# The-Learning-And-Vision-Atelier-LAVA/BUFFER

Hardware: AMD Instinct MI355X
Metric: registration pairs/sec (higher is better)
Workload: dtype f32

## Files before the change

buffer_amd/_lib.py:

```python
import ctypes as C
import os

_HERE = os.path.dirname(os.path.abspath(__file__))
LIB_PATH = os.environ.get("BUF_LIB_PATH") or os.path.join(_HERE, "libbuffer_hip.so")

BUF_OK = 0


class BufferHipError(RuntimeError):
    pass


class buf_grid_t(C.Structure):
    _fields_ = [
        ("ws", C.c_void_p), ("ws_bytes", C.c_size_t),
        ("ns", C.c_int), ("nb", C.c_int),
        ("cells_per_elem", C.c_int64),
        ("radius", C.c_float),
        ("supports", C.c_void_p),
        ("desc", C.c_void_p), ("s_off", C.c_void_p), ("table", C.c_void_p),
        ("sorted", C.c_void_p), ("order", C.c_void_p), ("scan_tmp", C.c_void_p),
    ]


# ... 37 lines not shown
    "buf_vn_gather_block_pre": (_i, [_vp, _vp, _vp, _vp, _i, _i, _i, _i, _i, _f, _vp, _vp, _vp, _vp, _f, _vp, _vp, _sz, _vp]),
    "buf_vn_pointwise": (_i, [_vp, _vp, _i, _i, _i, _vp, _i, _i, _i, _vp, _vp, _vp, _vp, _f, _vp, _vp, _vp]),
    "buf_gather_max": (_i, [_vp, _vp, _i, _i, _i, _i, _vp, _vp]),
    "buf_vn_std": (_i, [_vp, _vp, _i, _i, _vp, _vp]),
    "buf_score_head_ws_bytes": (_sz, [_i, _i]),
    "buf_score_head": (_i, [_vp, _i, _vp, _i, _vp, _vp, _vp, _vp, _f, _vp, _vp, _vp, _vp, _f, _vp, _vp, _vp, _vp, _vp, _i, _vp, _vp, _i, _f,
                            _vp, _vp, _sz, _vp]),
    "buf_patch_voxelize_ws_bytes": (_sz, [_i]),
    "buf_patch_voxelize": (_i, [_vp, _vp, _i, _i, _f, _vp, _i, _i, _vp, _f, _i, _vp, _vp, _vp, _vp, _vp, _vp, _vp,
                                _vp, _vp, _sz, _vp]),
    "buf_cylindrical_net_wg": (_i, [_vp, _i, _vp, _vp, _vp, _vp, _vp, _vp, _vp]),
    "buf_cylindrical_net_wg_supports": (_i, [_vp, _vp]),
    "buf_cylindrical_net_split_safe": (_i, [_vp, _i, _vp, _vp, _vp, _vp, _vp, _vp, _vp, _vp, _vp, _vp, _vp, _vp]),
    "buf_cost_volume_net_split_safe": (_i, [_vp, _vp, _i, _vp, _vp, _i, _vp, _vp, _vp, _vp, _vp, _vp, _vp, _vp]),
    "buf_cylindrical_net_split": (_i, [_vp, _i, _vp, _vp, _vp, _vp, _vp, _vp, _vp, _vp]),
    "buf_cylindrical_net_split_head": (_i, [_vp, _i, _vp, _vp, _vp, _vp, _vp, _vp, _vp, _vp, _vp, _vp]),
    "buf_split_gemm_count": (C.c_longlong, [_i, _i, _i, _i]),
    "buf_split_tile_gemm": (_i, [_vp, _i, _i, _i, _i, _vp]),
    "buf_cost_volume_net_split": (_i, [_vp, _vp, _i, _vp, _vp, _vp, _vp, _vp]),
    "buf_cost_volume_net_split_gather": (_i, [_vp, _i, _vp, _vp, _i, _vp, _vp, _vp, _vp, _vp]),
    "buf_split_filter_count": (C.c_longlong, [_i, _i]),
    "buf_split_tile_filters": (_i, [_vp, _i, _i, _vp]),
    "buf_winograd_tile_weights": (_i, [_vp, _i, _i, _vp]),
    "buf_winograd_group": (_i, [_i, _i]),
    "buf_cost_winograd_group": (_i, [_i]),
    "buf_winograd_tile_filters": (_i, [_vp, _i, _i, _i, _i, _vp]),
    "buf_voxel_downsample_ws_bytes": (_sz, [_i, _i64]),
    "buf_voxel_downsample": (_i, [_vp, _vp, _i, _i, C.c_double, _vp, _vp, _vp, _i64, _vp, _sz, _vp]),
    "buf_voxel_downsample_batch_ws_bytes": (_sz, [_i, _i, _i64]),
    "buf_voxel_downsample_batch": (_i, [_vp, _i, _i, _vp, _i, C.c_double, _vp, _vp, _i64, _vp, _sz, _vp]),
    "buf_knn_normals": (_i, [_vp, _i, _vp, _i, _vp, _i, _i, _vp, _i, _vp, _vp, _vp]),
    "buf_icp_ws_bytes": (_sz, [_i, _i, _i, _i]),
    "buf_icp_batched": (_i, [_vp, _vp, _vp, _vp, _vp, _i, _i, _f, _vp, _i, C.c_double, C.c_double, _vp, _vp, _vp, _vp, _vp,
                             _vp, _sz, _vp]),
    "buf_pair_stats_ws_bytes": (_sz, [_i, _i, _i, _i, _i64]),
    "buf_pair_stats": (_i, [_vp, _vp, _i, _vp, _vp, _i, _vp, _f, _i64, _vp, _vp, _vp, _vp, _sz, _vp]),
    "buf_match_metrics": (_i, [_vp, _vp, _vp, _i, _i, _vp, _vp, _f, _f, _f, _vp, _vp, _vp]),
    "buf_row_linear": (_i, [_vp, _i, _i, _i, _vp, _vp, _i, _vp, _vp]),
    "buf_segment_instance_norm_ws_bytes": (_sz, [_i, _i]),
    "buf_segment_instance_norm": (_i, [_vp, _i, _i, _vp, _i, _f, _vp, _vp, _sz, _vp]),
    "buf_descriptor_head": (_i, [_vp, _i, _vp, _vp, _vp, _vp]),
    "buf_cost_volume_net": (_i, [_vp, _vp, _i, _vp, _vp, _vp, _vp]),
    "buf_cost_volume_net_gather": (_i, [_vp, _i, _vp, _vp, _i, _vp, _vp, _vp, _vp]),
    "buf_hypotheses_score": (_i, [_vp, _vp, _vp, _vp, _vp, _i, _i, _f, _vp, _vp, _vp, _vp, _vp, _vp]),
    "buf_ransac_ws_bytes": (_sz, [_i]),
    "buf_ransac_kabsch": (_i, [_vp, _vp, _vp, _i, _i, C.c_uint64, _f, _f, _vp, _vp, _vp, _sz, _vp]),
# ... 34 lines not shown
```

buffer_amd/csrc/buffer_hip.hip:

```cpp
#include <stdlib.h>
#include "core.hip"
#include "radius.hip"
#include "icp.hip"
#include "pairstats.hip"
#include "metrics.hip"
#include "subsample.hip"
#include "pointops.hip"
#include "vn.hip"
#include "voxelize.hip"
#include "registration.hip"
#include "convnet.hip"
#include "convnet_h3.hip"
#include "costnet_h3.hip"
#include "preprocess.hip"
#include "convnet_wg.hip"
#include "costnet.hip"
#include "split_safe.hip"
```

buffer_amd/csrc/convnet_wg.hip:

```cpp
#include "common.h"
#include <type_traits>

#define WG_CS 160
#define WG_ROW 22
#define WG_ZERO 154
#define WG_MAXC 128
#define WG_LAYERS 8
#define WG_THREADS 256
#define WG_BUF (WG_MAXC * WG_CS)
#define WG_KSTEP (16 * WG_CS)
#define WG_BLOCKS 16

typedef float wgf4 __attribute__((ext_vector_type(4)));
typedef float wgf2 __attribute__((ext_vector_type(2)));
typedef const __attribute__((address_space(3))) wgf2* wg_lds_f2;

struct CylWgParams {
    const float* wt[WG_LAYERS];
    const float* bias[WG_LAYERS];
    int cin[WG_LAYERS], cout[WG_LAYERS], relu[WG_LAYERS];
    const int* only_if;
#ifdef WG_STAMP
    long long* stamps;
#endif
// ... 464 lines not shown
    wg_first_weights<2, 0, 2>(rs, wp, lofs, wstride, W1);
    float park[2][3][16];
    wg_round<2, 0, 2>(RA, rs, wp, wp, lofs, k4 >> 2, wstride, pstride, bv, W1, Y);
    wg_park<0>(Y, park);
    wg_park<1>(Y, park);
    wgf4 Yb[2];
    wg_round_direct<2>(RA[2][0], rs, wp, lofs, k4 >> 2, wstride, pstride, bv, W1, Yb);
    Y[0][2][0][0] = Yb[0]; Y[1][2][0][0] = Yb[1];
    wg_park<2>(Y, park);
    __syncthreads();
    int lane_s = threadIdx.x & (WAVE - 1);
    asm volatile("" : "+v"(lane_s));
#pragma unroll
    for (int n = 0; n < 2; n++) {
#pragma unroll
        for (int t = 0; t < 3; t++)
#pragma unroll
            for (int q = 0; q < (t == 2 ? 4 : 16); q++)
                asm volatile("v_accvgpr_read_b32 %0, %1" : "=v"(Y[n][t][q >> 3][(q >> 2) & 1][q & 3]) : "a"(park[n][t][q]));
        wg_store(Y[n], 2 * pair + n, relu, act, lane_s & 15, lane_s >> 4);
    }
}

__device__ __forceinline__ void cyl_net_wg_body(const float* __restrict__ x, const CylWgParams& P, float* __restrict__ y, float* __restrict__ lds)
{
    float* act = lds;
    const int patch = blockIdx.x;
    const int w = __builtin_amdgcn_readfirstlane(threadIdx.x / WAVE);
    WG_STAMP_AT(17)
#ifdef WG_STAMP
    if (threadIdx.x == 0) { P.stamps[(size_t)gridDim.x * 80 + blockIdx.x * 4 + 0] = __builtin_amdgcn_s_memtime(); P.stamps[(size_t)gridDim.x * 80 + blockIdx.x * 4 + 1] = __builtin_amdgcn_s_memrealtime(); }
#endif
    {
        const wgf4* src = reinterpret_cast<const wgf4*>(x + (size_t)patch * P.cin[0] * 140);
        const int nq = P.cin[0] * 35;
        wgf4 v[8];
#pragma unroll
        for (int k = 0; k < 8; k++) {
            const int i = threadIdx.x + k * WG_THREADS;
            if (i < nq) v[k] = __builtin_nontemporal_load(src + i);
        }
        auto put = [&](int i, wgf4 u) __attribute__((always_inline)) {
            const int c = i / 35, q = i - c * 35;
            const int row = q / 5, col = (q - row * 5) * 4;
            float* p = act + c * WG_CS + row * WG_ROW + col + 1;
            p[0] = u[0]; p[1] = u[1]; p[2] = u[2]; p[3] = u[3];
            if (col == 0) p[20] = u[0];
            if (col == 16) p[-17] = u[3];
        };
#pragma unroll
        for (int k = 0; k < 8; k++) {
            const int i = threadIdx.x + k * WG_THREADS;
            if (i < nq) put(i, v[k]);
        }
        for (int i = threadIdx.x + 8 * WG_THREADS; i < nq; i += WG_THREADS) put(i, __builtin_nontemporal_load(src + i));
    }
    for (int i = threadIdx.x; i < WG_MAXC * 4; i += WG_THREADS) act[(i >> 2) * WG_CS + WG_ZERO + (i & 3)] = 0.f;
    __syncthreads();
    WG_STAMP_AT(0)
    WgAddrPark pk;
    {
        int lane0 = threadIdx.x & (WAVE - 1);
        asm volatile("" : "+v"(lane0));
        wg_park_addresses(act, lane0 & 15, lane0 >> 4, pk);
    }
#pragma unroll 1
    for (int l = 0; l < WG_LAYERS; l++) {
        const int cin = P.cin[l], cout = P.cout[l];
        if (cout == 128) wg_layer_pair(act, P.wt[l], P.bias[l], cin, cout, P.relu[l], w, pk);
        else if (cout == 64) wg_layer_msplit(act, P.wt[l], P.bias[l], cin, cout, P.relu[l], w, pk);
        else if (l < WG_LAYERS - 1) wg_layer_mksplit<false>(act, nullptr, P.wt[l], P.bias[l], cin, cout, P.relu[l], w, pk);
        else wg_layer_mksplit<true>(act, y + (size_t)patch * cout * 140, P.wt[l], P.bias[l], cin, cout, P.relu[l], w, pk);
        WG_STAMP_AT(2 * l + 1)
        __syncthreads();
        WG_STAMP_AT(2 * l + 2)
    }
#ifdef WG_STAMP
    if (threadIdx.x == 0) { P.stamps[(size_t)gridDim.x * 80 + blockIdx.x * 4 + 2] = __builtin_amdgcn_s_memtime(); P.stamps[(size_t)gridDim.x * 80 + blockIdx.x * 4 + 3] = __builtin_amdgcn_s_memrealtime(); }
#endif
}

// ... 47 lines not shown
{
    for (int l = 0; l < WG_LAYERS; l++) {
        const int ci = cin[l], co = cout[l];
        BUF_REQUIRE(ci > 0 && ci % 16 == 0 && ci <= WG_MAXC && (co == 32 || co == 64 || co == 128), BUF_EINVAL,
                    "buf_cylindrical_net_wg: layer %d has unsupported widths %d -> %d", l, ci, co);
        BUF_REQUIRE(co != 128 || ci % 32 == 0, BUF_EINVAL,
                    "buf_cylindrical_net_wg: layer %d has unsupported widths %d -> %d (128 output channels need Cin %% 32 == 0)", l, ci, co);
        BUF_REQUIRE(co != 32 || (ci % 32 == 0 && ci <= 64), BUF_EINVAL,
                    "buf_cylindrical_net_wg: layer %d has unsupported widths %d -> %d (32 output channels need Cin = 32 or 64)", l, ci, co);
        BUF_REQUIRE(l == 0 || ci == cout[l - 1], BUF_EINVAL, "buf_cylindrical_net_wg: layer %d width mismatch", l);
        BUF_REQUIRE(l == 0 || cout[l - 1] != 32 || co == 32, BUF_EINVAL,
                    "buf_cylindrical_net_wg: layer %d has unsupported widths %d -> %d (only 32-output layers may follow a 32-output layer)", l, ci, co);
    }
    BUF_REQUIRE(cout[WG_LAYERS - 1] == 32, BUF_EINVAL, "buf_cylindrical_net_wg: the last layer must have 32 channels");
    return BUF_OK;
}

extern "C" int buf_cylindrical_net_wg_supports(const int* cin_host, const int* cout_host)
{
    BUF_REQUIRE(cin_host && cout_host, BUF_EINVAL, "buf_cylindrical_net_wg_supports: null argument");
    return wg_check_widths(cin_host, cout_host);
}

static int wg_launch(const float* x, int npatch, const float* const* wt_host, const float* const* bias_host, const int* cin_host,
                     const int* cout_host, const int* relu_host, float* y, const int* only_if, void* stream)
{
    BUF_REQUIRE(npatch >= 0, BUF_EINVAL, "buf_cylindrical_net_wg: npatch=%d", npatch);
    if (npatch == 0) return BUF_OK;
    BUF_REQUIRE(x && y && wt_host && bias_host && cin_host && cout_host && relu_host, BUF_EINVAL, "buf_cylindrical_net_wg: null argument");
    CylWgParams P;
    for (int l = 0; l < WG_LAYERS; l++) {
        P.wt[l] = wt_host[l]; P.bias[l] = bias_host[l];
        P.cin[l] = cin_host[l]; P.cout[l] = cout_host[l]; P.relu[l] = relu_host[l];
        BUF_REQUIRE(P.wt[l] && P.bias[l], BUF_EINVAL, "buf_cylindrical_net_wg: null weights for layer %d", l);
    }
    if (int rc = wg_check_widths(P.cin, P.cout)) return rc;
    P.only_if = only_if;
    size_t lds = sizeof(float) * WG_BUF;
    static LdsGrant grant, grant_rerun;
    if (int rc = only_if ? grant_dynamic_lds((const void*)k_cyl_net_wg_rerun, lds, grant_rerun) : grant_dynamic_lds((const void*)k_cyl_net_wg, lds, grant)) return rc;
    double macs = 0;
    for (int l = 0; l < WG_LAYERS; l++) macs += 9.0 * P.cin[l] * P.cout[l];
    TimedSpan span;
    bool timed = !only_if && timing_begin((hipStream_t)stream, &span, 2.0 * 140 * macs * npatch, BUF_TIMED_CYL_NET);
#ifdef WG_STAMP
    BUF_CHECK_HIP(hipMalloc(&P.stamps, (size_t)npatch * (4 * 20 + 4) * sizeof(long long)));
#endif
    if (only_if) k_cyl_net_wg_rerun<<<npatch, WG_THREADS, lds, (hipStream_t)stream>>>(x, P, y);
    else k_cyl_net_wg<<<npatch, WG_THREADS, lds, (hipStream_t)stream>>>(x, P, y);
    if (timed) timing_end((hipStream_t)stream, &span);
    BUF_LAUNCH_CHECK();
#ifdef WG_STAMP
    {
        BUF_CHECK_HIP(hipStreamSynchronize((hipStream_t)stream));
        long long* h = (long long*)malloc((size_t)npatch * (4 * 20 + 4) * sizeof(long long));
        BUF_CHECK_HIP(hipMemcpy(h, P.stamps, (size_t)npatch * (4 * 20 + 4) * sizeof(long long), hipMemcpyDeviceToHost));
        double comp[WG_LAYERS][4] = {}, wait[WG_LAYERS][4] = {}, tot = 0, pre = 0; long n = 0;
        for (int b = npatch / 2; b < npatch; b++, n++)
            for (int w = 0; w < 4; w++) {
                const long long* q = h + ((size_t)b * 4 + w) * 20;
// ... 27 lines not shown
```

buffer_amd/csrc/split_safe.hip:

```cpp
#include "common.h"

extern "C" int buf_cylindrical_net_split_safe(const float* x, int npatch, const void* const* wt_split_host, const float* const* wt_wg_host,
                                              const float* const* bias_host, const int* cin_host, const int* cout_host, const int* relu_host,
                                              const float* head_params, float* y_or_equi, float* desc, int* status_dev, int* flags_ws,
                                              void* stream)
{
    BUF_REQUIRE(npatch >= 0, BUF_EINVAL, "buf_cylindrical_net_split_safe: npatch=%d", npatch);
    if (npatch == 0) return BUF_OK;
    BUF_REQUIRE(x && y_or_equi && flags_ws && wt_split_host && wt_wg_host && bias_host && cin_host && cout_host && relu_host, BUF_EINVAL,
                "buf_cylindrical_net_split_safe: null argument");
    BUF_REQUIRE(!head_params || desc, BUF_EINVAL, "buf_cylindrical_net_split_safe: head without desc");
    if (int rc = buf_cylindrical_net_wg_supports(cin_host, cout_host)) return rc;
    hipStream_t s = (hipStream_t)stream;
    BUF_CHECK_HIP(hipMemsetAsync(flags_ws, 0, sizeof(int) * (size_t)npatch, s));
    int rc = h3_launch(x, npatch, wt_split_host, bias_host, cin_host, cout_host, relu_host, head_params ? nullptr : y_or_equi, head_params,
                       desc, head_params ? y_or_equi : nullptr, status_dev, stream, flags_ws);
    if (rc) return rc;
    rc = wg_launch(x, npatch, wt_wg_host, bias_host, cin_host, cout_host, relu_host, y_or_equi, flags_ws, stream);
    if (rc) return rc;
    if (head_params) {
        k_desc_head_masked<<<npatch, DH_THREADS, 0, s>>>(y_or_equi, head_params, desc, y_or_equi, flags_ws);
        BUF_LAUNCH_CHECK();
    }
    return BUF_OK;
}

extern "C" int buf_cost_volume_net_split_safe(const float* s_eq, const float* t_eq, int ele_n, const long long* s_rows, const long long* t_rows,
                                              int m, const void* const* wt_split_host, const float* const* bias_split_host,
                                              const float* const* wt_f32_host, const float* const* bias_f32_host, float* ind_out,
                                              int* status_dev, int* flags_ws, void* stream)
{
    BUF_REQUIRE(m >= 0, BUF_EINVAL, "buf_cost_volume_net_split_safe: m=%d", m);
    if (m == 0) return BUF_OK;
    BUF_REQUIRE(s_eq && t_eq && wt_split_host && bias_split_host && wt_f32_host && bias_f32_host && ind_out && flags_ws, BUF_EINVAL,
                "buf_cost_volume_net_split_safe: null argument");
    BUF_REQUIRE((s_rows == nullptr) == (t_rows == nullptr), BUF_EINVAL, "buf_cost_volume_net_split_safe: one row list without the other");
    BUF_REQUIRE(!s_rows || ele_n == 7, BUF_EINVAL, "buf_cost_volume_net_split_safe: ele_n=%d (the kernels are built for ele_n = 7)", ele_n);
    hipStream_t s = (hipStream_t)stream;
// ... 7 lines not shown
```

buffer_amd/ops.py:

```python
import ctypes as C
import time
import os
import numpy as np
import torch

from . import _lib
from ._lib import buf_grid_t, check


def _stream():
    return C.c_void_p(torch.cuda.current_stream().cuda_stream)


def _dev(t, dtype, what):
    if not isinstance(t, torch.Tensor) or not t.is_cuda:
        raise _lib.BufferHipError(f"{what}: expected a tensor in device memory (buffer_amd has no CPU path)")
    if t.dtype != dtype:
        t = t.to(dtype)
    return t.contiguous()


def _ptr(t):
    return C.c_void_p(t.data_ptr()) if t is not None else C.c_void_p(0)

# ... 543 lines not shown
    return poses


def mfma_tile_weights(wt, lk_major=False):
    K, cout = wt.shape
    assert K % 16 == 0 and cout % 16 == 0
    t = wt.reshape(K // 16, 4, 4, cout // 16, 16)
    perm = (0, 3, 1, 4, 2) if lk_major else (0, 3, 2, 4, 1)
    return np.ascontiguousarray(np.transpose(t, perm), dtype=np.float32).reshape(-1)


def winograd_tile_weights(w, ng=None, blocks=4):
    cout, cin = w.shape[0], w.shape[1]
    assert cin % 4 == 0 and cout % 16 == 0
    if ng is None:
        ng = _lib.lib().buf_winograd_group(cin, cout)
    G = np.array([[1, 0, 0], [.5, .5, .5], [.5, -.5, .5], [0, 0, 1]], np.float64)
    G5 = np.concatenate([G, [[0, 1, 0]]])
    U = np.einsum('ia,ocab,jb->ijoc', G5, np.asarray(w, np.float64), G)
    U = U[:blocks].reshape(blocks, 4, cout // (16 * ng), ng, 16, cin // 4, 4)
    return np.ascontiguousarray(np.transpose(U, (2, 0, 5, 3, 6, 4, 1)), dtype=np.float32).reshape(-1)


class CylindricalNet:

    def __init__(self, layers, device):
        self.wt, self.bias, self.cin, self.cout, self.relu = [], [], [], [], []
        self.entry = "buf_cylindrical_net_wg"
        for w, b, relu in layers:
            cout, cin = w.shape[0], w.shape[1]
            self.wt.append(torch.from_numpy(winograd_tile_weights(w)).to(device))
            self.bias.append(torch.from_numpy(np.ascontiguousarray(b, dtype=np.float32)).to(device))
            self.cin.append(cin); self.cout.append(cout); self.relu.append(1 if relu else 0)
        n = len(layers)
        self._wp = (C.c_void_p * n)(*[t.data_ptr() for t in self.wt])
        self._bp = (C.c_void_p * n)(*[t.data_ptr() for t in self.bias])
        self._ci = (C.c_int * n)(*self.cin)
        self._co = (C.c_int * n)(*self.cout)
        self._re = (C.c_int * n)(*self.relu)

    def __call__(self, x):
        L = _lib.lib()
        x = x.contiguous()
        P = x.shape[0]
        y = torch.empty((P, self.cout[-1], 7, 20), dtype=torch.float32, device=x.device)
        check(L.buf_cylindrical_net_wg(_ptr(x), P, self._wp, self._bp, self._ci, self._co, self._re, _ptr(y), _stream()), self.entry)
        return y


def split_tile_filters(w):
    L = _lib.lib()
    w = np.ascontiguousarray(w, dtype=np.float32)
    cout, cin = w.shape[0], w.shape[1]
    out = np.empty(L.buf_split_filter_count(cout, cin), dtype=np.uint16)
    check(L.buf_split_tile_filters(w.ctypes.data, cout, cin, out.ctypes.data), "buf_split_tile_filters")
    return out


class CylindricalNetSplit:

    def __init__(self, layers, device):
        self.wt, self.bias, self.cin, self.cout, self.relu = [], [], [], [], []
        self.entry = "buf_cylindrical_net_split"
        for w, b, relu in layers:
            cout, cin = w.shape[0], w.shape[1]
            self.wt.append(torch.from_numpy(split_tile_filters(w).view(np.int16)).to(device))
            self.bias.append(torch.from_numpy(np.ascontiguousarray(b, dtype=np.float32)).to(device))
            self.cin.append(cin); self.cout.append(cout); self.relu.append(1 if relu else 0)
        n = len(layers)
        self.status = torch.zeros(1, dtype=torch.int32, device=device)
        self._wp = (C.c_void_p * n)(*[t.data_ptr() for t in self.wt])
        self._bp = (C.c_void_p * n)(*[t.data_ptr() for t in self.bias])
        self._ci = (C.c_int * n)(*self.cin)
        self._co = (C.c_int * n)(*self.cout)
        self._re = (C.c_int * n)(*self.relu)
        self.last_flags = None
        self.safe = n == 8 and _lib.lib().buf_cylindrical_net_wg_supports(self._ci, self._co) == 0 and not os.environ.get('BUF_SPLIT_UNSAFE')
        if self.safe:
            self.wt_wg = [torch.from_numpy(winograd_tile_weights(w)).to(device) for w, _, _ in layers]
            self._wwp = (C.c_void_p * n)(*[t.data_ptr() for t in self.wt_wg])

    def _safe_call(self, x, head):
        L = _lib.lib()
        x = x.contiguous()
        P = x.shape[0]
        out = torch.empty((P, self.cout[-1], 7, 20), dtype=torch.float32, device=x.device)
        desc = torch.empty((P, 32), dtype=torch.float32, device=x.device) if head is not None else None
        self.last_flags = torch.empty((max(P, 1),), dtype=torch.int32, device=x.device)
        check(L.buf_cylindrical_net_split_safe(_ptr(x), P, self._wp, self._wwp, self._bp, self._ci, self._co, self._re,
                                               _ptr(head.params) if head is not None else None, _ptr(out), _ptr(desc), _ptr(self.status),
                                               _ptr(self.last_flags), _stream()), "buf_cylindrical_net_split_safe")
        return (desc, out) if head is not None else out

    def __call__(self, x):
        if self.safe:
            return self._safe_call(x, None)
        L = _lib.lib()
        x = x.contiguous()
        P = x.shape[0]
        y = torch.empty((P, self.cout[-1], 7, 20), dtype=torch.float32, device=x.device)
        check(L.buf_cylindrical_net_split(_ptr(x), P, self._wp, self._bp, self._ci, self._co, self._re, _ptr(y), _ptr(self.status), _stream()),
              self.entry)
        return y

    def with_head(self, x, head):
        if self.safe:
            return self._safe_call(x, head)
        L = _lib.lib()
        x = x.contiguous()
        P = x.shape[0]
        desc = torch.empty((P, 32), dtype=torch.float32, device=x.device)
        equi = torch.empty((P, 32, 7, 20), dtype=torch.float32, device=x.device)
# ... 185 lines not shown
```

include/buffer_hip.h:

```cpp
#ifndef BUFFER_HIP_H
#define BUFFER_HIP_H
#include <stddef.h>
#include <stdint.h>
#ifdef __cplusplus
extern "C" {
#endif

#define BUF_OK            0
#define BUF_EINVAL       -1
#define BUF_EHIP         -2
#define BUF_EWORKSPACE   -3
#define BUF_ECAPACITY    -4
#define BUF_ENODEVICE    -5

const char* buf_last_error(void);
int         buf_version(void);
int         buf_device_count(void);
#define BUF_TIMED_GRID_QUERY 0
#define BUF_TIMED_CYL_NET    1
#define BUF_TIMED_COST_NET   2
#define BUF_TIMED_SELECT_PATCHES 3
#define BUF_TIMED_PATCH_VOXELIZE 4
#define BUF_TIMED_FPS            5
#define BUF_TIMED_NN1            6
// ... 85 lines not shown
                       void* stream);
size_t  buf_segment_instance_norm_ws_bytes(int nseg, int c);
int     buf_segment_instance_norm(const float* x, int n, int c, const int* lens_host, int nseg, float eps, float* out,
                                  void* ws, size_t ws_bytes, void* stream);
int     buf_vn_std(const float* x, const float* z, int n, int c, float* out, void* stream);
size_t  buf_score_head_ws_bytes(int n, int nseg);
int     buf_score_head(const float* x, int n, const int* lens_host, int nseg,
                       const float* vn1_wf, const float* vn1_wd, const float* vn1_bsc, const float* vn1_bsh, float vn1_slope,
                       const float* vn2_wf, const float* vn2_wd, const float* vn2_bsc, const float* vn2_bsh, float vn2_slope,
                       const float* lin, const float* w0, const float* b0, const float* w1, const float* b1, int c1,
                       const float* w2, const float* b2, int final_activation, float eps, float* out,
                       void* ws, size_t ws_bytes, void* stream);

size_t  buf_patch_voxelize_ws_bytes(int ncentres);
int     buf_patch_voxelize(const float* patches, const float* axis, int npatch, int npts, float des_r,
                           const float* centres, int ncentres, int azi_n, const float* azi_cs, float voxel_r,
                           int nsample, const float* mlp_w_host, const float* mlp_b_host, const float* bn_scale_host,
                           const float* bn_shift_host, float* out_x, float* out_R, float* out_rand, float* out_patches,
                           void* ws, size_t ws_bytes, void* stream);

int     buf_winograd_group(int cin, int cout);
int     buf_winograd_tile_weights(const float* w_host, int cout, int cin, float* out_host);
int     buf_winograd_tile_filters(const float* w_host, int cout, int cin, int ng, int nblk, float* out_host);
int     buf_cylindrical_net_wg(const float* x, int npatch, const float* const* wt_host, const float* const* bias_host,
                               const int* cin_host, const int* cout_host, const int* relu_host, float* y, void* stream);
int     buf_cylindrical_net_wg_supports(const int* cin_host, const int* cout_host);

long long buf_split_filter_count(int cout, int cin);
int     buf_split_tile_filters(const float* w_host, int cout, int cin, unsigned short* out_host);
int     buf_cylindrical_net_split(const float* x, int npatch, const void* const* wt_host, const float* const* bias_host,
                                  const int* cin_host, const int* cout_host, const int* relu_host, float* y, int* status_dev, void* stream);
int     buf_cylindrical_net_split_head(const float* x, int npatch, const void* const* wt_host, const float* const* bias_host,
                                       const int* cin_host, const int* cout_host, const int* relu_host, const float* head_params,
                                       float* desc, float* equi, int* status_dev, void* stream);

int     buf_cylindrical_net_split_safe(const float* x, int npatch, const void* const* wt_split_host, const float* const* wt_wg_host,
                                       const float* const* bias_host, const int* cin_host, const int* cout_host, const int* relu_host,
                                       const float* head_params, float* y_or_equi, float* desc, int* status_dev, int* flags_ws, void* stream);

int     buf_descriptor_head(const float* y, int npatch, const float* params, float* desc, float* equi, void* stream);

int     buf_cost_winograd_group(int layer);
int     buf_cost_volume_net(const float* s_eq, const float* t_eq, int m, const float* const* wt_host,
                            const float* const* bias_host, float* ind_out, void* stream);
int     buf_cost_volume_net_gather(const float* equi, int ele_n, const long long* s_rows, const long long* t_rows, int m,
                                   const float* const* wt_host, const float* const* bias_host, float* ind_out, void* stream);
// ... 71 lines not shown
```

Baseline: 154.2.

## Add Winograd F(2x2,4x3)-style kernel path for 128-channel cylindrical conv layers

```diff
diff --git a/buffer_amd/_lib.py b/buffer_amd/_lib.py
--- a/buffer_amd/_lib.py
+++ b/buffer_amd/_lib.py
@@ -83,6 +83,7 @@
     "buf_split_filter_count": (C.c_longlong, [_i, _i]),
     "buf_split_tile_filters": (_i, [_vp, _i, _i, _vp]),
     "buf_winograd_tile_weights": (_i, [_vp, _i, _i, _vp]),
+    "buf_winograd_f24_tile_weights": (_i, [_vp, _i, _i, _vp]),
     "buf_winograd_group": (_i, [_i, _i]),
     "buf_cost_winograd_group": (_i, [_i]),
     "buf_winograd_tile_filters": (_i, [_vp, _i, _i, _i, _i, _vp]),
diff --git a/buffer_amd/csrc/buffer_hip.hip b/buffer_amd/csrc/buffer_hip.hip
--- a/buffer_amd/csrc/buffer_hip.hip
+++ b/buffer_amd/csrc/buffer_hip.hip
@@ -14,5 +14,6 @@
 #include "costnet_h3.hip"
 #include "preprocess.hip"
 #include "convnet_wg.hip"
+#include "convnet_w24.hip"
 #include "costnet.hip"
 #include "split_safe.hip"
diff --git a/buffer_amd/csrc/convnet_w24.hip b/buffer_amd/csrc/convnet_w24.hip
--- /dev/null
+++ b/buffer_amd/csrc/convnet_w24.hip
@@ -0,0 +1,418 @@
+#include "common.h"
+
+#define W24_WSTRIDE 768
+#define W24_SET_F22(CIN) (16 * 128 * (CIN))
+
+__device__ __forceinline__ void w24_tile(int li, int& ty, int& tx)
+{
+    const bool last = li == 15;
+    ty = last ? 3 : li / 5;
+    tx = last ? 4 : li - 5 * ty;
+}
+
+__device__ __forceinline__ unsigned w24_row_addr(unsigned act_addr, int a, int li, int lk)
+{
+    int ty, tx;
+    w24_tile(li, ty, tx);
+    const int row = 2 * ty - 1 + a;
+    return act_addr + 4u * (unsigned)(lk * WG_CS + ((row >= 0 && row <= 6) ? row * WG_ROW + 4 * tx : WG_ZERO));
+}
+
+struct W24AddrPark { float a[4]; };
+__device__ __forceinline__ void w24_park_addresses(const float* act, int li, int lk, W24AddrPark& pk)
+{
+    const unsigned act_addr = (unsigned)(size_t)(__attribute__((address_space(3))) const float*)act;
+#pragma unroll
+    for (int a = 0; a < 4; a++) {
+        const unsigned v = w24_row_addr(act_addr, a, li, lk);
+        asm volatile("v_accvgpr_write_b32 %0, %1" : "=a"(pk.a[a]) : "v"(v));
+    }
+}
+
+#define W24_LOAD(DST, A0, A1_, OFS)                                                                       \
+    {                                                                                                     \
+        _Pragma("unroll") for (int q_ = 0; q_ < 3; q_++) {                                                \
+            DST[q_] = *(wg_lds_f2)(size_t)((A0) + (OFS) + 8 * q_);                                        \
+            asm volatile("" : "+v"(A0));                                                                  \
+        }                                                                                                 \
+        _Pragma("unroll") for (int q_ = 0; q_ < 3; q_++) {                                                \
+            DST[3 + q_] = *(wg_lds_f2)(size_t)((A1_) + (OFS) + 8 * q_);                                   \
+            asm volatile("" : "+v"(A1_));                                                                 \
+        }                                                                                                 \
+    }
+
+__device__ __forceinline__ wgf2 w24_ldw2(__amdgpu_buffer_rsrc_t rs, unsigned uniform_float_ofs, unsigned lane_byte_ofs)
+{
+    return __builtin_bit_cast(wgf2, __builtin_amdgcn_raw_buffer_load_b64(rs, lane_byte_ofs, uniform_float_ofs * 4, 0));
+}
+
+#define W24_U(n, k, j) ((j) < 3 ? W4[n][k][j] : ((j) == 5 ? W4[n][k][3] : W2[n][k][(j) - 3]))
+
+template <int I, bool PRIMED, int INEXT>
+__device__ __forceinline__ void w24_pass(unsigned (&RA)[4], __amdgpu_buffer_rsrc_t rs, unsigned wp, unsigned wp_next, unsigned lofs4, unsigned lofs2,
+                                         int niter, wgf4 (&W4)[2][2], wgf2 (&W2)[2][2], wgf4 (&acc)[2][6], wgf2 (&D)[2][6])
+{
+    constexpr int A1 = wg_a1(I), A2 = wg_a2(I);
+    constexpr int A1N = wg_a1(INEXT < 0 ? 0 : INEXT), A2N = wg_a2(INEXT < 0 ? 0 : INEXT);
+    float V[2][6];
+    unsigned P0 = RA[A1], P1 = RA[A2];
+    if constexpr (!PRIMED) {
+        W24_LOAD(D[0], P0, P1, 0)
+        W24_LOAD(D[1], P0, P1, WG_KSTEP)
+    }
+#define W24_XFORM(BUF)                                                                                    \
+    {                                                                                                     \
+        float r_[6];                                                                                      \
+        _Pragma("unroll") for (int b = 0; b < 6; b++) {                                                   \
+            const float da_ = D[BUF][b >> 1][b & 1];                                                      \
+            const float db_ = D[BUF][3 + (b >> 1)][b & 1];                                                \
+            r_[b] = I == 1 ? wg_add(da_, db_) : (I == 2 ? wg_sub(db_, da_) : wg_sub(da_, db_));           \
+        }                                                                                                 \
+        const float c_ = wg_sub(r_[4], r_[2]), e_ = wg_sub(r_[3], r_[1]);                                 \
+        const float a_ = __builtin_fmaf(-4.f, r_[2], r_[4]), b_ = __builtin_fmaf(-4.f, r_[1], r_[3]);     \
+        V[BUF][0] = __builtin_fmaf(4.f, r_[0], __builtin_fmaf(-4.f, r_[2], c_));                          \
+        V[BUF][1] = wg_add(a_, b_); V[BUF][2] = wg_sub(a_, b_);                                           \
+        V[BUF][3] = __builtin_fmaf(2.f, e_, c_); V[BUF][4] = __builtin_fmaf(-2.f, e_, c_);                \
+        V[BUF][5] = __builtin_fmaf(-4.f, e_, wg_sub(r_[5], r_[3]));                                       \
+    }
+    W24_XFORM(0)
+#pragma unroll 1
+    for (int it = 0; it < niter; it++) {
+        const bool more = it + 1 < niter;
+        const unsigned wcur = wp + 4 * it * W24_WSTRIDE;
+        const unsigned wn = more ? wcur + 4 * W24_WSTRIDE : wp_next;
+        const unsigned adv = more ? 4u * WG_KSTEP : 0u;
+        __builtin_amdgcn_sched_barrier(0);
+#pragma unroll
+        for (int s = 0; s < 4; s++) {
+            if (s < 2) W24_LOAD(D[s & 1], P0, P1, (s + 2) * WG_KSTEP)
+            else {
+                if (s == 2) { P0 += adv; P1 += adv; }
+                if constexpr (INEXT >= 0) {
+                    unsigned q0 = more ? P0 : RA[A1N], q1 = more ? P1 : RA[A2N];
+                    W24_LOAD(D[s & 1], q0, q1, (s - 2) * WG_KSTEP)
+                } else
+                    W24_LOAD(D[s & 1], P0, P1, (s - 2) * WG_KSTEP)
+            }
+            __builtin_amdgcn_sched_barrier(0);
+#pragma unroll
+            for (int n = 0; n < 2; n++)
+#pragma unroll
+                for (int j = 0; j < 6; j++)
+                    acc[n][j] = __builtin_amdgcn_mfma_f32_16x16x4f32(W24_U(n, s & 1, j), V[s & 1][j], acc[n][j], 0, 0, 0);
+            __builtin_amdgcn_sched_barrier(0);
+            W24_XFORM((s + 1) & 1)
+#pragma unroll
+            for (int n = 0; n < 2; n++) {
+                const unsigned o = s < 2 ? wcur + (s + 2) * W24_WSTRIDE : wn + (s - 2) * W24_WSTRIDE;
+                W4[n][s & 1] = wg_ldw(rs, o + n * 256, lofs4);
+                W2[n][s & 1] = w24_ldw2(rs, o + 512 + n * 128, lofs2);
+            }
+            __builtin_amdgcn_sched_barrier(0);
+        }
+    }
+#undef W24_XFORM
+}
+
+__device__ __forceinline__ void w24_round(unsigned (&RA)[4], __amdgpu_buffer_rsrc_t rs, unsigned wp, unsigned wp_after, unsigned lofs4, unsigned lofs2,
+                                          int niter, unsigned pstride, const float* __restrict__ bias_lane, wgf4 (&W4)[2][2], wgf2 (&W2)[2][2],
+                                          wgf4 (&Y)[2][2][4])
+{
+    using std::integral_constant;
+    wgf2 D[2][6];
+    wgf4 bv[2];
+#pragma unroll
+    for (int n = 0; n < 2; n++) bv[n] = *reinterpret_cast<const wgf4*>(bias_lane + n * 16);
+    wgf4 acc[2][6];
+    float zero = 0.f;
+    asm volatile("" : "+v"(zero));
+#pragma unroll
+    for (int n = 0; n < 2; n++)
+#pragma unroll
+        for (int j = 0; j < 6; j++) acc[n][j] = (wgf4){ zero, zero, zero, zero };
+    auto run = [&](auto ic) __attribute__((always_inline)) {
+        constexpr int I = decltype(ic)::value;
+        constexpr int INEXT = I == 3 ? 0 : I + 1;
+        if constexpr (I == 1) {
+#pragma unroll
+            for (int n = 0; n < 2; n++) acc[n][1] += bv[n];
+        }
+        constexpr int ICHAIN = (INEXT != 0 && wg_chains(I)) ? INEXT : -1;
+        w24_pass<I, wg_chains(I - 1), ICHAIN>(RA, rs, wp + I * pstride, INEXT == 0 ? wp_after : wp + (I + 1) * pstride, lofs4, lofs2, niter, W4, W2, acc, D);
+        __builtin_amdgcn_sched_barrier(0);
+#pragma unroll
+        for (int n = 0; n < 2; n++) {
+            wgf4 f[4];
+#pragma unroll
+            for (int r = 0; r < 4; r++) {
+                const float p = acc[n][1][r] + acc[n][2][r], q = acc[n][1][r] - acc[n][2][r];
+                const float t = acc[n][3][r] + acc[n][4][r], d = acc[n][3][r] - acc[n][4][r];
+                f[0][r] = acc[n][0][r] + p + t;
+                f[1][r] = __builtin_fmaf(2.f, d, q);
+                f[2][r] = __builtin_fmaf(4.f, t, p);
+                f[3][r] = __builtin_fmaf(8.f, d, q) + acc[n][5][r];
+            }
+#pragma unroll
+            for (int v = 0; v < 4; v++) {
+                if constexpr (I == 0) Y[n][1][v] = f[v];
+                else if constexpr (I == 1) {
+#pragma unroll
+                    for (int r = 0; r < 4; r++) Y[n][1][v][r] = __builtin_fmaf(2.f, f[v][r], -Y[n][1][v][r]);
+                }
+                else if constexpr (I == 2) Y[n][0][v] = f[v];
+                else Y[n][1][v] -= f[v];
+                if constexpr (I == 2) asm volatile("" : "+v"(Y[n][0][v]));
+                else asm volatile("" : "+v"(Y[n][1][v]));
+            }
+        }
+    };
+    run(integral_constant<int, 0>{});
+    run(integral_constant<int, 1>{});
+    run(integral_constant<int, 2>{});
+    run(integral_constant<int, 3>{});
+}
+
+__device__ __forceinline__ void w24_round_direct(unsigned row5, __amdgpu_buffer_rsrc_t rs, unsigned wp, unsigned lofs, int niter, unsigned pstride,
+                                                 const float* __restrict__ bias_lane, wgf4 (&W4)[2][2], wgf4 (&Y)[2])
+{
+    constexpr int wstride = W24_WSTRIDE;
+    wgf4 Wr[3][2][2];
+#pragma unroll
+    for (int n = 0; n < 2; n++)
+#pragma unroll
+        for (int k = 0; k < 2; k++) {
+            Wr[0][n][k] = W4[n][k];
+            Wr[1][n][k] = wg_ldw(rs, wp + pstride + n * 256 + k * wstride, lofs);
+            Wr[2][n][k] = wg_ldw(rs, wp + 2 * pstride + n * 256 + k * wstride, lofs);
+        }
+    float X[2][6];
+    unsigned pa = row5;
+    WG_LOADD(X[0], pa, 0)
+    WG_LOADD(X[1], pa, WG_KSTEP)
+    wgf4 acc[2][3];
+    float zero = 0.f;
+    asm volatile("" : "+v"(zero));
+#pragma unroll
+    for (int n = 0; n < 2; n++) {
+        acc[n][0] = (wgf4){ zero, zero, zero, zero };
+        acc[n][1] = (wgf4){ zero, zero, zero, zero };
+        acc[n][2] = *reinterpret_cast<const wgf4*>(bias_lane + n * 16);
+    }
+    float G[2][6];
+#define W24_TAPS(SLOT)                                                                                    \
+    _Pragma("unroll") for (int n = 0; n < 2; n++) {                                                       \
+        const wgf4 u0_ = Wr[0][n][SLOT], u1_ = Wr[1][n][SLOT], u2_ = Wr[2][n][SLOT];                      \
+        const float d1_ = wg_sub(u1_[1], u2_[1]), d2_ = wg_sub(u1_[2], u2_[2]);                           \
+        G[n][0] = u0_[0]; G[n][1] = wg_sub(u0_[1], u0_[2]); G[n][2] = u0_[3];                             \
+        G[n][3] = wg_sub(u1_[0], u2_[0]); G[n][4] = wg_sub(d1_, d2_); G[n][5] = wg_sub(u1_[3], u2_[3]);   \
+    }
+#define W24_RELOAD(SLOT, OFS)                                                                             \
+    _Pragma("unroll") for (int n = 0; n < 2; n++)                                                         \
+        _Pragma("unroll") for (int blk = 0; blk < 3; blk++) Wr[blk][n][SLOT] = wg_ldw(rs, (OFS) + blk * pstride + n * 256, lofs);
+    W24_TAPS(0)
+    W24_RELOAD(0, wp + 2 * wstride)
+#pragma unroll 1
+    for (int it = 0; it < niter; it++) {
+        const bool more = it + 1 < niter;
+        const unsigned wcur = wp + 4 * it * wstride;
+        const unsigned wn = more ? wcur + 4 * wstride : wp;
+        const unsigned adv = more ? 4u * WG_KSTEP : 0u;
+        __builtin_amdgcn_sched_barrier(0);
+#pragma unroll
+        for (int s = 0; s < 4; s++) {
+#pragma unroll
+            for (int b = 0; b < 3; b++)
+#pragma unroll
+                for (int a = 0; a < 2; a++)
+#pragma unroll
+                    for (int n = 0; n < 2; n++)
+                        acc[n][b] = __builtin_amdgcn_mfma_f32_16x16x4f32(G[n][a * 3 + b], X[s & 1][a * 3 + b], acc[n][b], 0, 0, 0);
+            __builtin_amdgcn_sched_barrier(0);
+            if (s < 2) WG_LOADD(X[s & 1], pa, (s + 2) * WG_KSTEP)
+            else {
+                if (s == 2) pa += adv;
+                WG_LOADD(X[s & 1], pa, (s - 2) * WG_KSTEP)
+            }
+            __builtin_amdgcn_sched_barrier(0);
+            W24_TAPS((s + 1) & 1)
+            if (s == 0) W24_RELOAD(1, wcur + 3 * wstride)
+            else W24_RELOAD((s + 1) & 1, wn + (s - 1) * wstride)
+            __builtin_amdgcn_sched_barrier(0);
+        }
+    }
+#undef W24_TAPS
+#undef W24_RELOAD
+#pragma unroll
+    for (int n = 0; n < 2; n++)
+#pragma unroll
+        for (int r = 0; r < 4; r++) Y[n][r] = __builtin_fmaf(4.f, acc[n][0][r], __builtin_fmaf(-3.f, acc[n][1][r], acc[n][2][r]));
+}
+
+__device__ __forceinline__ void w24_store_tile(const wgf4 (&Yt)[2][4], int nt, int relu, float* __restrict__ act, int li, int lk)
+{
+    const int n0 = nt * 16 + lk * 4;
+    const float lo = relu ? 0.f : -__builtin_inff();
+    int ty, tx;
+    w24_tile(li, ty, tx);
+#pragma unroll
+    for (int u = 0; u < 2; u++) {
+        const int row = 2 * ty + u;
+        const bool ok = row < 7;
+        int pos[4];
+#pragma unroll
+        for (int v = 0; v < 4; v++) pos[v] = ok ? row * WG_ROW + 4 * tx + 1 + v : WG_ZERO + 4;
+        const int h0 = (ok && tx == 0) ? row * WG_ROW + 21 : WG_ZERO + 4;
+        const int h1 = (ok && tx == 4) ? row * WG_ROW : WG_ZERO + 5;
+        float* p = act + n0 * WG_CS;
+#pragma unroll
+        for (int r = 0; r < 4; r++) {
+            float val[4];
+#pragma unroll
+            for (int v = 0; v < 4; v++) { val[v] = fmaxf(Yt[u][v][r], lo); p[r * WG_CS + pos[v]] = val[v]; }
+            p[r * WG_CS + h0] = val[0]; p[r * WG_CS + h1] = val[3];
+        }
+    }
+}
+
+__device__ __forceinline__ void w24_layer_pair(float* __restrict__ act, const float* __restrict__ wt, const float* __restrict__ bias, int cin, int relu,
+                                               int pair, const WgAddrPark& pk, const W24AddrPark& pk24)
+{
+    act[(threadIdx.x >> 1) * WG_CS + WG_ZERO + 4 + (threadIdx.x & 1)] = 0.f;
+    __syncthreads();
+    int lane = threadIdx.x & (WAVE - 1);
+    asm volatile("" : "+v"(lane));
+    const int lk = lane >> 4;
+    const int k4 = cin >> 2;
+    unsigned RA[4];
+#pragma unroll
+    for (int a = 0; a < 4; a++) asm volatile("v_accvgpr_read_b32 %0, %1" : "=v"(RA[a]) : "a"(pk24.a[a]));
+    const unsigned row5 = wg_parked(pk, 2, 0);
+    const __amdgpu_buffer_rsrc_t rs = wg_weights(wt);
+    const unsigned pstride = (unsigned)(k4 * W24_WSTRIDE);
+    const unsigned wp = (unsigned)pair * 4 * pstride;
+    const unsigned lofs4 = lane * 16, lofs2 = lane * 8;
+    const float* bv = bias + (2 * pair) * 16 + lk * 4;
+    wgf4 W4[2][2];
+    wgf2 W2[2][2];
+#pragma unroll
+    for (int n = 0; n < 2; n++)
+#pragma unroll
+        for (int k = 0; k < 2; k++) {
+            W4[n][k] = wg_ldw(rs, wp + k * W24_WSTRIDE + n * 256, lofs4);
+            W2[n][k] = w24_ldw2(rs, wp + k * W24_WSTRIDE + 512 + n * 128, lofs2);
+        }
+    wgf4 Y[2][2][4];
+    float park[2][36];
+    w24_round(RA, rs, wp, wp, lofs4, lofs2, k4 >> 2, pstride, bv, W4, W2, Y);
+#pragma unroll
+    for (int n = 0; n < 2; n++)
+#pragma unroll
+        for (int q = 0; q < 32; q++) asm volatile("v_accvgpr_write_b32 %0, %1" : "=a"(park[n][q]) : "v"(Y[n][q >> 4][(q >> 2) & 3][q & 3]));
+    wgf4 Yb[2];
+    w24_round_direct(row5, rs, wp, lofs4, k4 >> 2, pstride, bv, W4, Yb);
+#pragma unroll
+    for (int n = 0; n < 2; n++)
+#pragma unroll
+        for (int q = 0; q < 4; q++) asm volatile("v_accvgpr_write_b32 %0, %1" : "=a"(park[n][32 + q]) : "v"(Yb[n][q]));
+    __syncthreads();
+    int lane_s = threadIdx.x & (WAVE - 1);
+    asm volatile("" : "+v"(lane_s));
+#pragma unroll
+    for (int n = 0; n < 2; n++) {
+#pragma unroll
+        for (int q = 0; q < 32; q++) asm volatile("v_accvgpr_read_b32 %0, %1" : "=v"(Y[n][q >> 4][(q >> 2) & 3][q & 3]) : "a"(park[n][q]));
+#pragma unroll
+        for (int q = 0; q < 4; q++) asm volatile("v_accvgpr_read_b32 %0, %1" : "=v"(Yb[n][q]) : "a"(park[n][32 + q]));
+        w24_store_tile(Y[n], 2 * pair + n, relu, act, lane_s & 15, lane_s >> 4);
+        wg_store_row6<false>(Yb[n], 2 * pair + n, relu, act, nullptr, lane_s & 15, lane_s >> 4);
+    }
+}
+
+__device__ __forceinline__ void cyl_net_w24_body(const float* __restrict__ x, const CylWgParams& P, float* __restrict__ y, float* __restrict__ lds)
+{
+    float* act = lds;
+    const int patch = blockIdx.x;
+    const int w = __builtin_amdgcn_readfirstlane(threadIdx.x / WAVE);
+    wg_load_input(x, P, act, patch);
+    WgAddrPark pk;
+    W24AddrPark pk24;
+    {
+        int lane0 = threadIdx.x & (WAVE - 1);
+        asm volatile("" : "+v"(lane0));
+        wg_park_addresses(act, lane0 & 15, lane0 >> 4, pk);
+        w24_park_addresses(act, lane0 & 15, lane0 >> 4, pk24);
+    }
+#pragma unroll 1
+    for (int l = 0; l < WG_LAYERS; l++) {
+        const int cin = P.cin[l], cout = P.cout[l];
+        if (cout == 128) w24_layer_pair(act, P.wt[l], P.bias[l], cin, P.relu[l], w, pk, pk24);
+        else if (cout == 64) wg_layer_msplit(act, P.wt[l], P.bias[l], cin, cout, P.relu[l], w, pk);
+        else if (l < WG_LAYERS - 1) wg_layer_mksplit<false>(act, nullptr, P.wt[l], P.bias[l], cin, cout, P.relu[l], w, pk);
+        else wg_layer_mksplit<true>(act, y + (size_t)patch * cout * 140, P.wt[l], P.bias[l], cin, cout, P.relu[l], w, pk);
+        __syncthreads();
+    }
+}
+
+__global__ void __launch_bounds__(WG_THREADS, 2) k_cyl_net_w24(const float* __restrict__ x, CylWgParams P, float* __restrict__ y)
+{
+    extern __shared__ float lds[];
+    cyl_net_w24_body(x, P, y, lds);
+}
+
+__global__ void __launch_bounds__(WG_THREADS, 2) k_cyl_net_w24_rerun(const float* __restrict__ x, CylWgParams P, float* __restrict__ y)
+{
+    extern __shared__ float lds[];
+    if (P.only_if[blockIdx.x] == 0) return;
+    cyl_net_w24_body(x, P, y, lds);
+}
+
+extern "C" int buf_winograd_f24_tile_weights(const float* w_host, int cout, int cin, float* out_host)
+{
+    BUF_REQUIRE(w_host && out_host, BUF_EINVAL, "buf_winograd_f24_tile_weights: null argument");
+    BUF_REQUIRE(cout > 0 && cin > 0 && cout % 32 == 0 && cin % 4 == 0, BUF_EINVAL, "buf_winograd_f24_tile_weights: widths %d -> %d", cin, cout);
+    static const double G2[4][3] = { { 1, 0, 0 }, { .5, .5, .5 }, { .5, -.5, .5 }, { 0, 0, 1 } };
+    const double s6 = 1.0 / 6, s12 = 1.0 / 12, s24 = 1.0 / 24;
+    const double G4[6][3] = { { .25, 0, 0 }, { -s6, -s6, -s6 }, { -s6, s6, -s6 }, { s24, s12, s6 }, { s24, -s12, s6 }, { 0, 0, 1 } };
+    const int k4 = cin / 4;
+    for (int o = 0; o < cout; o++)
+        for (int c = 0; c < cin; c++) {
+            const float* g = w_host + ((size_t)o * cin + c) * 9;
+            const int n = o / 16, lane = (c % 4) * 16 + o % 16;
+            for (int i = 0; i < 4; i++) {
+                float* blk = out_host + (((size_t)(n / 2) * 4 + i) * k4 + c / 4) * W24_WSTRIDE;
+                for (int j = 0; j < 6; j++) {
+                    double u = 0;
+                    for (int a = 0; a < 3; a++)
+                        for (int b = 0; b < 3; b++) u += G2[i][a] * (double)g[3 * a + b] * G4[j][b];
+                    if (j == 3 || j == 4) blk[512 + (n % 2) * 128 + lane * 2 + (j - 3)] = (float)u;
+                    else blk[(n % 2) * 256 + lane * 4 + (j == 5 ? 3 : j)] = (float)u;
+                }
+            }
+        }
+    return BUF_OK;
+}
+
+static int w24_launch(const float* x, int npatch, CylWgParams P, float* y, void* stream)
+{
+    for (int l = 0; l < WG_LAYERS; l++) {
+        const bool flag = (P.relu[l] & WG_F24_FLAG) != 0;
+        BUF_REQUIRE(P.relu[l] >= 0 && P.relu[l] <= (WG_F24_FLAG | 1), BUF_EINVAL, "buf_cylindrical_net_wg: layer %d has relu flags %d", l, P.relu[l]);
+        BUF_REQUIRE(flag == (P.cout[l] == 128), BUF_EINVAL,
+                    "buf_cylindrical_net_wg: the F(2x4) flag goes on every layer with 128 output channels and on no other (layer %d: %d -> %d, flags %d)",
+                    l, P.cin[l], P.cout[l], P.relu[l]);
+        if (flag) P.wt[l] += W24_SET_F22(P.cin[l]);
+        P.relu[l] &= 1;
+    }
+    size_t lds = sizeof(float) * WG_BUF;
+    static LdsGrant grant, grant_rerun;
+    if (int rc = P.only_if ? grant_dynamic_lds((const void*)k_cyl_net_w24_rerun, lds, grant_rerun) : grant_dynamic_lds((const void*)k_cyl_net_w24, lds, grant)) return rc;
+    double macs = 0;
+    for (int l = 0; l < WG_LAYERS; l++) macs += 9.0 * P.cin[l] * P.cout[l];
+    TimedSpan span;
+    bool timed = !P.only_if && timing_begin((hipStream_t)stream, &span, 2.0 * 140 * macs * npatch, BUF_TIMED_CYL_NET);
+    if (P.only_if) k_cyl_net_w24_rerun<<<npatch, WG_THREADS, lds, (hipStream_t)stream>>>(x, P, y);
+    else k_cyl_net_w24<<<npatch, WG_THREADS, lds, (hipStream_t)stream>>>(x, P, y);
+    if (timed) timing_end((hipStream_t)stream, &span);
+    BUF_LAUNCH_CHECK();
+    return BUF_OK;
+}
diff --git a/buffer_amd/csrc/convnet_wg.hip b/buffer_amd/csrc/convnet_wg.hip
--- a/buffer_amd/csrc/convnet_wg.hip
+++ b/buffer_amd/csrc/convnet_wg.hip
@@ -510,15 +510,8 @@
     }
 }
 
-__device__ __forceinline__ void cyl_net_wg_body(const float* __restrict__ x, const CylWgParams& P, float* __restrict__ y, float* __restrict__ lds)
-{
-    float* act = lds;
-    const int patch = blockIdx.x;
-    const int w = __builtin_amdgcn_readfirstlane(threadIdx.x / WAVE);
-    WG_STAMP_AT(17)
-#ifdef WG_STAMP
-    if (threadIdx.x == 0) { P.stamps[(size_t)gridDim.x * 80 + blockIdx.x * 4 + 0] = __builtin_amdgcn_s_memtime(); P.stamps[(size_t)gridDim.x * 80 + blockIdx.x * 4 + 1] = __builtin_amdgcn_s_memrealtime(); }
-#endif
+__device__ __forceinline__ void wg_load_input(const float* __restrict__ x, const CylWgParams& P, float* __restrict__ act, int patch)
+{
     {
         const wgf4* src = reinterpret_cast<const wgf4*>(x + (size_t)patch * P.cin[0] * 140);
         const int nq = P.cin[0] * 35;
@@ -545,6 +538,18 @@
     }
     for (int i = threadIdx.x; i < WG_MAXC * 4; i += WG_THREADS) act[(i >> 2) * WG_CS + WG_ZERO + (i & 3)] = 0.f;
     __syncthreads();
+}
+
+__device__ __forceinline__ void cyl_net_wg_body(const float* __restrict__ x, const CylWgParams& P, float* __restrict__ y, float* __restrict__ lds)
+{
+    float* act = lds;
+    const int patch = blockIdx.x;
+    const int w = __builtin_amdgcn_readfirstlane(threadIdx.x / WAVE);
+    WG_STAMP_AT(17)
+#ifdef WG_STAMP
+    if (threadIdx.x == 0) { P.stamps[(size_t)gridDim.x * 80 + blockIdx.x * 4 + 0] = __builtin_amdgcn_s_memtime(); P.stamps[(size_t)gridDim.x * 80 + blockIdx.x * 4 + 1] = __builtin_amdgcn_s_memrealtime(); }
+#endif
+    wg_load_input(x, P, act, patch);
     WG_STAMP_AT(0)
     WgAddrPark pk;
     {
@@ -638,6 +643,10 @@
     return wg_check_widths(cin_host, cout_host);
 }
 
+#define WG_F24_FLAG BUF_CYL_F24
+static inline bool wg_f24_flagged(int relu) { return relu == WG_F24_FLAG || relu == (WG_F24_FLAG | 1); }
+static int w24_launch(const float* x, int npatch, CylWgParams P, float* y, void* stream);
+
 static int wg_launch(const float* x, int npatch, const float* const* wt_host, const float* const* bias_host, const int* cin_host,
                      const int* cout_host, const int* relu_host, float* y, const int* only_if, void* stream)
 {
@@ -652,6 +661,8 @@
     }
     if (int rc = wg_check_widths(P.cin, P.cout)) return rc;
     P.only_if = only_if;
+    for (int l = 0; l < WG_LAYERS; l++)
+        if (wg_f24_flagged(relu_host[l])) return w24_launch(x, npatch, P, y, stream);
     size_t lds = sizeof(float) * WG_BUF;
     static LdsGrant grant, grant_rerun;
     if (int rc = only_if ? grant_dynamic_lds((const void*)k_cyl_net_wg_rerun, lds, grant_rerun) : grant_dynamic_lds((const void*)k_cyl_net_wg, lds, grant)) return rc;
diff --git a/buffer_amd/csrc/split_safe.hip b/buffer_amd/csrc/split_safe.hip
--- a/buffer_amd/csrc/split_safe.hip
+++ b/buffer_amd/csrc/split_safe.hip
@@ -13,7 +13,9 @@
     if (int rc = buf_cylindrical_net_wg_supports(cin_host, cout_host)) return rc;
     hipStream_t s = (hipStream_t)stream;
     BUF_CHECK_HIP(hipMemsetAsync(flags_ws, 0, sizeof(int) * (size_t)npatch, s));
-    int rc = h3_launch(x, npatch, wt_split_host, bias_host, cin_host, cout_host, relu_host, head_params ? nullptr : y_or_equi, head_params,
+    int relu_split[WG_LAYERS];
+    for (int l = 0; l < WG_LAYERS; l++) relu_split[l] = wg_f24_flagged(relu_host[l]) ? (relu_host[l] & 1) : relu_host[l];
+    int rc = h3_launch(x, npatch, wt_split_host, bias_host, cin_host, cout_host, relu_split, head_params ? nullptr : y_or_equi, head_params,
                        desc, head_params ? y_or_equi : nullptr, status_dev, stream, flags_ws);
     if (rc) return rc;
     rc = wg_launch(x, npatch, wt_wg_host, bias_host, cin_host, cout_host, relu_host, y_or_equi, flags_ws, stream);
diff --git a/buffer_amd/ops.py b/buffer_amd/ops.py
--- a/buffer_amd/ops.py
+++ b/buffer_amd/ops.py
@@ -589,14 +589,53 @@
     return np.ascontiguousarray(np.transpose(U, (2, 0, 5, 3, 6, 4, 1)), dtype=np.float32).reshape(-1)
 
 
+def winograd_f24_tile_weights(w):
+    cout, cin = w.shape[0], w.shape[1]
+    assert cin % 4 == 0 and cout % 32 == 0
+    U = winograd_f24_filters(w)
+    U = U.reshape(4, 6, cout // 32, 2, 16, cin // 4, 4)
+    U = np.transpose(U, (2, 0, 5, 3, 6, 4, 1))
+    lead = U.shape[:3]
+    wide = U[..., [0, 1, 2, 5]].reshape(*lead, 512)
+    narrow = U[..., [3, 4]].reshape(*lead, 256)
+    return np.ascontiguousarray(np.concatenate([wide, narrow], axis=-1), dtype=np.float32).reshape(-1)
+
+
+F24_G2 = np.array([[1, 0, 0], [.5, .5, .5], [.5, -.5, .5], [0, 0, 1]], np.float64)
+F24_G4 = np.array([[.25, 0, 0], [-1 / 6, -1 / 6, -1 / 6], [-1 / 6, 1 / 6, -1 / 6], [1 / 24, 1 / 12, 1 / 6], [1 / 24, -1 / 12, 1 / 6], [0, 0, 1]],
+                  np.float64)
+
+
+def winograd_f24_filters(w):
+    w64 = np.asarray(w, np.float64)
+    U = np.zeros((4, 6) + w64.shape[:2], np.float64)
+    for a in range(3):
+        for b in range(3):
+            U += (F24_G2[:, a][:, None, None, None] * w64[None, None, :, :, a, b]) * F24_G4[:, b][None, :, None, None]
+    return U
+
+
+F24_FLAG = 2
+
+
+def cyl_layer_filters(w):
+    wt = winograd_tile_weights(w)
+    if w.shape[0] != 128:
+        return wt, 0
+    return np.concatenate([wt, winograd_f24_tile_weights(w)]), F24_FLAG
+
+
 class CylindricalNet:
 
-    def __init__(self, layers, device):
+    def __init__(self, layers, device, f24=True):
         self.wt, self.bias, self.cin, self.cout, self.relu = [], [], [], [], []
         self.entry = "buf_cylindrical_net_wg"
+        flags = []
         for w, b, relu in layers:
             cout, cin = w.shape[0], w.shape[1]
-            self.wt.append(torch.from_numpy(winograd_tile_weights(w)).to(device))
+            wt, flag = cyl_layer_filters(w) if f24 else (winograd_tile_weights(w), 0)
+            flags.append(flag)
+            self.wt.append(torch.from_numpy(wt).to(device))
             self.bias.append(torch.from_numpy(np.ascontiguousarray(b, dtype=np.float32)).to(device))
             self.cin.append(cin); self.cout.append(cout); self.relu.append(1 if relu else 0)
         n = len(layers)
@@ -604,7 +643,7 @@
         self._bp = (C.c_void_p * n)(*[t.data_ptr() for t in self.bias])
         self._ci = (C.c_int * n)(*self.cin)
         self._co = (C.c_int * n)(*self.cout)
-        self._re = (C.c_int * n)(*self.relu)
+        self._re = (C.c_int * n)(*[r | f for r, f in zip(self.relu, flags)])
 
     def __call__(self, x):
         L = _lib.lib()
@@ -644,8 +683,10 @@
         self.last_flags = None
         self.safe = n == 8 and _lib.lib().buf_cylindrical_net_wg_supports(self._ci, self._co) == 0 and not os.environ.get('BUF_SPLIT_UNSAFE')
         if self.safe:
-            self.wt_wg = [torch.from_numpy(winograd_tile_weights(w)).to(device) for w, _, _ in layers]
+            tiled = [cyl_layer_filters(w) for w, _, _ in layers]
+            self.wt_wg = [torch.from_numpy(wt).to(device) for wt, _ in tiled]
             self._wwp = (C.c_void_p * n)(*[t.data_ptr() for t in self.wt_wg])
+            self._re_safe = (C.c_int * n)(*[r | f for r, (_, f) in zip(self.relu, tiled)])
 
     def _safe_call(self, x, head):
         L = _lib.lib()
@@ -654,7 +695,7 @@
         out = torch.empty((P, self.cout[-1], 7, 20), dtype=torch.float32, device=x.device)
         desc = torch.empty((P, 32), dtype=torch.float32, device=x.device) if head is not None else None
         self.last_flags = torch.empty((max(P, 1),), dtype=torch.int32, device=x.device)
-        check(L.buf_cylindrical_net_split_safe(_ptr(x), P, self._wp, self._wwp, self._bp, self._ci, self._co, self._re,
+        check(L.buf_cylindrical_net_split_safe(_ptr(x), P, self._wp, self._wwp, self._bp, self._ci, self._co, self._re_safe,
                                                _ptr(head.params) if head is not None else None, _ptr(out), _ptr(desc), _ptr(self.status),
                                                _ptr(self.last_flags), _stream()), "buf_cylindrical_net_split_safe")
         return (desc, out) if head is not None else out
diff --git a/include/buffer_hip.h b/include/buffer_hip.h
--- a/include/buffer_hip.h
+++ b/include/buffer_hip.h
@@ -131,6 +131,8 @@
 int     buf_winograd_group(int cin, int cout);
 int     buf_winograd_tile_weights(const float* w_host, int cout, int cin, float* out_host);
 int     buf_winograd_tile_filters(const float* w_host, int cout, int cin, int ng, int nblk, float* out_host);
+#define BUF_CYL_F24 2
+int     buf_winograd_f24_tile_weights(const float* w_host, int cout, int cin, float* out_host);
 int     buf_cylindrical_net_wg(const float* x, int npatch, const float* const* wt_host, const float* const* bias_host,
                                const int* cin_host, const int* cout_host, const int* relu_host, float* y, void* stream);
 int     buf_cylindrical_net_wg_supports(const int* cin_host, const int* cout_host);
```

Measured after the change: 162.6, median of 6. +5.5%, better.
